# eth-cscs/COSTA

Measured on AMD Instinct MI355X. Metric: GB/s device-resident tile pack+transpose+unpack (fp64), % HBM peak, higher is better.
Workload: dtype f64; 1 GPU; pxtran fp64 16384x16384, 256x256 blocks, op T, alpha=1 beta=0, 1x1 grid (BASELINE configs[1]); op=T, parallelism=1 rank(s), one per GPU, RCCL send/recv exchange, m=16384, n=16384, block=256, grid=1x1

## Files before the change

### costa_amd/__init__.py

```python
from __future__ import annotations

import ctypes as C
import os
import struct
from dataclasses import dataclass
from typing import Iterable, Sequence

import numpy as np

__all__ = [
    "CostaError", "lib", "FLOAT", "DOUBLE", "CFLOAT", "CDOUBLE", "INT32", "dtype_code",
    "np_dtype", "Layout", "block_cyclic_layout", "custom_layout", "Comm", "transform",
    "transform_batch", "transform_async", "transform_batch_async", "synchronize", "transformer", "copy_and_transform", "execute_tiles", "execute_tiles_mixed",
    "convert_subtile", "TileOp",
    "plan_export", "set_profiling", "get_stats", "release_caches", "TILE_OP_DTYPE",
]

FLOAT, DOUBLE, CFLOAT, CDOUBLE, INT32 = 0, 1, 2, 3, 4
_NP = {FLOAT: np.float32, DOUBLE: np.float64, CFLOAT: np.complex64,
       CDOUBLE: np.complex128, INT32: np.int32}

TILE_TRANSPOSE, TILE_CONJ, TILE_VEC_SRC, TILE_VEC_DST = 0x1, 0x2, 0x4, 0x8
SCALE_BITCOPY, SCALE_ZERO, SCALE_ALPHA, SCALE_AXPBY = 0, 1, 2, 3

# ... 99 lines not shown
        "costa_hip_layout_num_blocks": (i, [vp]),
        "costa_hip_layout_block": (i, [vp, i, C.POINTER(i), C.POINTER(i), C.POINTER(i),
                                       C.POINTER(i), C.POINTER(vp), C.POINTER(i)]),
        "costa_hip_comm_self": (i, [i, C.POINTER(vp)]),
        "costa_hip_comm_unique_id": (i, [C.c_char_p]),
        "costa_hip_comm_create": (i, [C.c_char_p, i, i, i, C.POINTER(vp)]),
        "costa_hip_comm_rank": (i, [vp]),
        "costa_hip_comm_size": (i, [vp]),
        "costa_hip_comm_destroy": (None, [vp]),
        "costa_hip_transform": (i, [vp, vp, c, vp, vp, vp]),
        "costa_hip_transform_batch": (i, [i, C.POINTER(vp), C.POINTER(vp), C.c_char_p, vp, vp,
                                          vp]),
        "costa_hip_transform_async": (i, [vp, vp, c, vp, vp, vp, vp]),
        "costa_hip_transform_batch_async": (i, [i, C.POINTER(vp), C.POINTER(vp), C.c_char_p, vp,
                                                vp, vp, vp]),
        "costa_hip_synchronize": (i, [vp]),
        "costa_hip_device_count": (i, [C.POINTER(i)]),
        "costa_hip_rccl_version": (i, [C.POINTER(i)]),
        "costa_hip_copy_and_transform": (i, [i, i, i, vp, i, i, vp, i, i, i, i, vp, vp]),
        "costa_hip_execute_tiles": (i, [i, C.POINTER(TileOp), i64, vp, vp, vp, i, i]),
        "costa_hip_execute_tiles_mixed": (i, [i, i, C.POINTER(TileOp), i64, vp, vp, vp, i, i]),
        "costa_hip_convert_subtile": (i, [i, i, C.POINTER(i), C.POINTER(i)]),
        "costa_hip_plan_export": (i, [i, C.POINTER(vp), C.POINTER(vp), C.c_char_p, vp, vp, i, i,
                                      C.POINTER(PlanInfo), vp, vp, vp, vp, vp, vp, vp, vp]),
        "costa_hip_set_profiling": (i, [i]),
        "costa_hip_get_stats": (i, [C.POINTER(FullStats), i]),
        "costa_hip_release_caches": (i, []),
        "costa_hip_set_host_staging": (i, [i]),
        "costa_hip_set_planner": (i, [i]),
        "costa_hip_plan_export_device": (i, [i, i, C.POINTER(vp), C.POINTER(vp), C.c_char_p, vp, vp,
                                             i, i, C.POINTER(PlanInfo), vp, vp, vp, vp, vp, vp, vp,
                                             vp]),
        "costa_hip_set_list_builder": (i, [i]),
        "costa_hip_work_export": (i, [i, vp, i64, i, i, vp, i64, vp, i64, C.POINTER(i64)]),
    }
    for name, (res, args) in sig.items():
        f = getattr(L, name)
        f.restype = res
        f.argtypes = args
    _lib = L
    return L


def _check(rc: int):
    if rc != 0:
        raise CostaError(rc, lib().costa_hip_last_error().decode(errors="replace"))


def _ptr(p) -> int:
    if p is None:
        return 0
    if isinstance(p, int):
        return p
    if isinstance(p, np.ndarray):
        return p.ctypes.data
    if hasattr(p, "data_ptr"):
        return p.data_ptr()
    raise TypeError(f"cannot take the address of {type(p)}")


def _scalar_bytes(code: int, x) -> bytes:
    if code == DOUBLE:
        return struct.pack("<d", float(x))
    if code == CDOUBLE:
        z = complex(x)
        return struct.pack("<dd", z.real, z.imag)
# ... 4 lines not shown
    return C.c_char(x.encode()[:1])


@dataclass
class BlockInfo:
    row_start: int
    row_end: int
    col_start: int
    col_end: int
    data: int
    ld: int


class Layout:

    def __init__(self, handle: int, dtype: int, keep: Iterable = ()):
        self._h = C.c_void_p(handle)
        self.dtype = dtype
        self._keep = list(keep)

    @property
    def handle(self) -> C.c_void_p:
        return self._h

    def num_blocks(self) -> int:
        return lib().costa_hip_layout_num_blocks(self._h)

    def block(self, i: int) -> BlockInfo:
        v = [C.c_int() for _ in range(4)]
        d, ld = C.c_void_p(), C.c_int()
        _check(lib().costa_hip_layout_block(self._h, i, *[C.byref(x) for x in v], C.byref(d),
                                            C.byref(ld)))
        return BlockInfo(v[0].value, v[1].value, v[2].value, v[3].value, d.value or 0, ld.value)

    def reorder_ranks(self, reordering: Sequence[int]):
        p = np.ascontiguousarray(reordering, dtype=np.int32)
        _check(lib().costa_hip_layout_reorder_ranks(self._h, p.ctypes.data_as(C.POINTER(C.c_int)),
                                                    int(p.size)))

    def close(self):
        if self._h and self._h.value:
            lib().costa_hip_layout_destroy(self._h)
            self._h = C.c_void_p(0)

    def __del__(self):
        try:
            self.close()
        except Exception:
            pass


def block_cyclic_layout(m, n, block_m, block_n, i, j, sub_m, sub_n, p_m, p_n, order, rsrc, csrc,
                        ptr, lld, ordering, rank, dtype=DOUBLE) -> Layout:
    code = dtype_code(dtype)
    h = C.c_void_p()
    _check(lib().costa_hip_block_cyclic_layout(code, m, n, block_m, block_n, i, j, sub_m, sub_n,
                                               p_m, p_n, _chr(order), rsrc, csrc,
                                               C.c_void_p(_ptr(ptr)), lld, _chr(ordering), rank,
                                               C.byref(h)))
    return Layout(h.value, code, [ptr])


def custom_layout(rowblocks, colblocks, rowsplit, colsplit, owners, localblocks, ordering,
                  dtype=DOUBLE) -> Layout:
    code = dtype_code(dtype)
    rs = np.ascontiguousarray(rowsplit, dtype=np.int32)
# ... 208 lines not shown
        def export(*args):
            return L.costa_hip_plan_export_device(int(device), *args)
    _check(export(n, a, c, tb, ab, bb, rank, nranks, C.byref(info), None, None,
                  None, None, None, None, None, None))
    lo = np.zeros(info.n_local, TILE_OP_DTYPE)
    po = np.zeros(info.n_pack, TILE_OP_DTYPE)
    uo = np.zeros(info.n_unpack, TILE_OP_DTYPE)
    cnt = [np.zeros(nranks, np.int64) for _ in range(4)]
    sc = np.zeros(2 * info.n_slots, _NP[code])
    _check(export(n, a, c, tb, ab, bb, rank, nranks, C.byref(info),
                  lo.ctypes.data, po.ctypes.data, uo.ctypes.data,
                  *[x.ctypes.data for x in cnt], sc.ctypes.data))
    return Plan(lo, po, uo, *cnt, sc, info.send_elems, info.recv_elems, info.local_elems)


def set_profiling(on: bool = True):
    _check(lib().costa_hip_set_profiling(int(on)))


def get_stats(reset: bool = False) -> dict:
    s = FullStats()
    _check(lib().costa_hip_get_stats(C.byref(s), int(reset)))
    return s.as_dict()


def release_caches():
    _check(lib().costa_hip_release_caches())


def set_planner(mode: int):
    _check(lib().costa_hip_set_planner(int(mode)))


def set_list_builder(mode: int):
    _check(lib().costa_hip_set_list_builder(int(mode)))


@dataclass
class WorkLists:
    ordered: np.ndarray
    work: np.ndarray
    meta: dict
    on_gpu: bool


_WORK_META = ("n_large", "n_medium", "n_skew", "n_cblock", "cblock_lds", "cb_map", "tiny_first",
              "n_tiny", "n_ordered", "n_work", "on_gpu", "flags")


def work_export(dtype, ops: np.ndarray, kind: str = "local", device=None) -> WorkLists:
    code = dtype_code(dtype)
    ops = np.ascontiguousarray(ops, dtype=TILE_OP_DTYPE)
    k = {"local": 0, "pack": 1, "unpack": 2}[kind]
    dev = -1 if device is None else int(device)
    meta = (C.c_int64 * 12)()
    L = lib()
    _check(L.costa_hip_work_export(code, ops.ctypes.data, ops.size, k, dev, None, 0, None, 0, meta))
    o = np.zeros(meta[8], TILE_OP_DTYPE)
    w = np.zeros(meta[9], np.uint64)
    _check(L.costa_hip_work_export(code, ops.ctypes.data, ops.size, k, dev, o.ctypes.data, o.size,
                                   w.ctypes.data, w.size, meta))
    m = dict(zip(_WORK_META, list(meta)))
    return WorkLists(o, w, m, bool(m["on_gpu"]))


def set_host_staging(mode: int):
# ... 8 lines not shown
```

### costa_amd/csrc/capi.cpp

```cpp
#include "engine.hpp"

#include <hip/hip_runtime.h>

#include <costa/transform.hpp>

#include <algorithm>
#include <cctype>
#include <complex>
#include <cstring>
#include <new>

struct costa_layout_s {
    costa::engine::elayout e;
    std::vector<int> base_owners;
};
struct costa_comm_s {
    costa::engine::comm* c = nullptr;
};

namespace {
thread_local std::string g_last_error;

template <typename F>
int guarded(F&& f) {
// ... 346 lines not shown
        [&](const std::vector<job>& jobs) { return costa::engine::make_plan(jobs, rank, nranks); },
        n, A, C, trans, alpha, beta, rank, nranks, info, local_ops, pack_ops, unpack_ops,
        send_counts, send_displs, recv_counts, recv_displs, scalars);
}

int costa_hip_plan_export_device(int device, int n, const costa_layout_t* A, const costa_layout_t* C,
                                 const char* trans, const void* alpha, const void* beta, int rank,
                                 int nranks, costa_plan_info_t* info, costa_tile_op_t* local_ops,
                                 costa_tile_op_t* pack_ops, costa_tile_op_t* unpack_ops,
                                 int64_t* send_counts, int64_t* send_displs, int64_t* recv_counts,
                                 int64_t* recv_displs, void* scalars) {
    device_restore keep;
    return export_plan(
        [&](const std::vector<job>& jobs) {
            auto p = costa::engine::make_plan_device(jobs, rank, nranks, 0, device, nullptr);
            if (!p)
                throw costa::engine::error(COSTA_ERR_ARG,
                                           "costa: the device planner does not apply to these "
                                           "layouts (local blocks are not exactly the rank's grid "
                                           "cells)");
            return p;
        },
        n, A, C, trans, alpha, beta, rank, nranks, info, local_ops, pack_ops, unpack_ops,
        send_counts, send_displs, recv_counts, recv_displs, scalars);
}

int costa_hip_set_planner(int mode) {
    return guarded([&] {
        if (mode < 0 || mode > 2) throw costa::engine::error(COSTA_ERR_ARG, "mode must be 0, 1 or 2");
        costa::engine::set_planner_mode(mode);
    });
}

int costa_hip_set_list_builder(int mode) {
    return guarded([&] {
        if (mode < 0 || mode > 2) throw costa::engine::error(COSTA_ERR_ARG, "mode must be 0, 1 or 2");
        costa::engine::set_list_builder_mode(mode);
    });
}

int costa_hip_work_export(int dtype, const costa_tile_op_t* ops, int64_t n_ops, int kind, int device,
                          costa_tile_op_t* ordered, int64_t cap_ordered, uint64_t* work,
                          int64_t cap_work, int64_t* meta) {
    auto body = [&] {
        if (!meta || (n_ops > 0 && !ops) || n_ops < 0) throw costa::engine::error(COSTA_ERR_ARG, "null argument");
        if (dtype < COSTA_FLOAT || dtype > COSTA_INT32) throw costa::engine::error(COSTA_ERR_ARG, "bad dtype");
        if (kind < 0 || kind > 2) throw costa::engine::error(COSTA_ERR_ARG, "kind must be 0, 1 or 2");
        std::vector<costa_tile_op_t> in(ops, ops + n_ops), o;
        std::vector<uint64_t> w;
        costa::engine::work_split ws;
        const bool on_gpu = costa::engine::work_export(
            costa_dtype_t(dtype), in, costa::engine::list_kind(kind), device, o, w, ws);
        const int64_t m[12] = {ws.n_large, ws.n_medium, ws.n_skew, ws.n_cblock, ws.cblock_lds, ws.cb_map,
                               ws.tiny_first, ws.n_tiny, int64_t(o.size()), int64_t(w.size()), on_gpu,
                               int64_t(ws.tr_shape) | int64_t(ws.sq) << 1 | int64_t(ws.full) << 2 |
                                   int64_t(ws.med_full) << 3 | int64_t(ws.med_sq) << 4 |
                                   int64_t(ws.skew_wide) << 5};
        std::memcpy(meta, m, sizeof(m));
        if (ordered && cap_ordered >= int64_t(o.size()) && !o.empty())
            std::memcpy(ordered, o.data(), o.size() * sizeof(o[0]));
        if (work && cap_work >= int64_t(w.size()) && !w.empty()) std::memcpy(work, w.data(), w.size() * sizeof(w[0]));
    };
    return device >= 0 ? gpu_guarded(body) : guarded(body);
}

int costa_hip_set_profiling(int on) {
// ... 138 lines not shown
```

### costa_amd/csrc/engine.cpp

```cpp
#include <exception>
#include <thread>
#include "engine.hpp"

#include <hip/hip_runtime.h>
#include <rccl/rccl.h>

#include <algorithm>
#include <numeric>
#include <chrono>
#include <cmath>
#include <cstdio>
#include <cstdlib>
#include <cstring>
#include <deque>
#include <list>
#include <map>
#include <mutex>
#include <unordered_map>

namespace costa {
namespace engine {

#define HIP_CHECK(x)                                                                   \
    do {                                                                               \
// ... 1347 lines not shown
        if (d) {
            hipDeviceptr_t base = nullptr;
            size_t sz = 0;
            if (hipMemGetAddressRange(&base, &sz, const_cast<char*>(b.data)) == hipSuccess) {
                lo = reinterpret_cast<uintptr_t>(base);
                hi = lo + sz;
            } else {
                (void)hipGetLastError();
            }
        }
    }
    return first;
}

}

namespace {
int g_host_mode = -1;
}
int host_staging_mode() {
    if (g_host_mode < 0) {
        const char* s = std::getenv("COSTA_HOST_STAGING");
        g_host_mode = s ? (std::atoi(s) != 0) : 1;
    }
    return g_host_mode;
}
void set_host_staging_mode(int mode) {
    std::lock_guard<std::recursive_mutex> lk(g_mutex);
    g_host_mode = mode != 0;
}

namespace {

struct hasher {
    uint64_t h = 0x9E3779B97F4A7C15ull;
    uint64_t h2 = 0x2545F4914F6CDD1Dull;
    void mix(uint64_t v) {
        v ^= v >> 33;
        v *= 0xff51afd7ed558ccdull;
        v ^= v >> 33;
        h = (h ^ v) * 0xc4ceb9fe1a85ec53ull + 0x165667b19e3779f9ull;
        h ^= h >> 29;
        h2 = (h2 + v) * 0x9fb21c651e98df25ull;
        h2 ^= h2 >> 31;
    }
    void mix_vec(const std::vector<int>& v) {
        mix(v.size());
        for (int x : v) mix(uint64_t(uint32_t(x)));
    }
    void mix_layout(const elayout& L) {
        mix(uint64_t(L.dtype));
        mix(uint64_t(uint8_t(L.ordering)));
        mix(uint64_t(L.n_ranks));
        mix_vec(L.rows_split);
        mix_vec(L.cols_split);
        mix_vec(L.owners);
        mix(L.blocks.size());
        for (const auto& b : L.blocks) {
            mix(uint64_t(uint32_t(b.rows.start)) | (uint64_t(uint32_t(b.rows.end)) << 32));
            mix(uint64_t(uint32_t(b.cols.start)) | (uint64_t(uint32_t(b.cols.end)) << 32));
            mix(reinterpret_cast<uintptr_t>(b.data));
            mix(uint64_t(uint32_t(b.ld)));
        }
    }
};

}

uint64_t layout_hash(const elayout& L) {
    hasher h;
    h.mix_layout(L);
    return h.h | 1;
}

void layout_hashes(const elayout& L, uint64_t& h1, uint64_t& h2) {
    hasher h;
    h.mix_layout(L);
    h1 = h.h | 1;
    h2 = h.h2;
}

void set_layout_hash(elayout& L) { layout_hashes(L, L.hash, L.hash2); }

namespace {

struct cached_plan {
    std::unique_ptr<plan> p;
    int device = 0;
    bool staged = false;
    std::vector<hrange> h2d_ranges, d2h_ranges;
    dbuf stage;
    dbuf d_local, w_local, d_scal;
    work_split l_local;
    bool tr_local = true, ax_local = true;
    convert_list c_local;
    struct xround {
        dbuf d_pack, w_pack, d_unpack, w_unpack;
        work_split l_pack, l_unpack;
        convert_list c_pack, c_unpack;
        bool tr_unpack = false, ax_unpack = false;
    };
    std::vector<std::unique_ptr<xround>> rounds;
    std::vector<unsigned char> scal_host;
    std::shared_ptr<host_pipeline> pipe;
};

constexpr size_t kMaxPlans = 16;
struct keyed_plan {
    uint64_t h = 0;
    std::vector<uint64_t> key;
    std::unique_ptr<cached_plan> plan;
};
std::list<keyed_plan> g_plans;

void key_layout(std::vector<uint64_t>& k, const elayout& L) {
    uint64_t h1 = L.hash, h2 = L.hash2;
    if (!h1) layout_hashes(L, h1, h2);
    k.push_back(h1);
    k.push_back(h2);
    k.push_back(uint64_t(L.dtype) | uint64_t(uint8_t(L.ordering)) << 8 |
                uint64_t(uint32_t(L.n_ranks)) << 32);
    k.push_back(uint64_t(uint32_t(L.nbr())) | uint64_t(uint32_t(L.nbc())) << 32);
    k.push_back(L.blocks.size());
    if (!L.blocks.empty())
        for (const eblock* b : {&L.blocks.front(), &L.blocks.back()}) {
            k.push_back(reinterpret_cast<uintptr_t>(b->data));
            k.push_back(uint64_t(uint32_t(b->ld)) | uint64_t(uint32_t(b->rows.start)) << 32);
        }
}

elayout remap(const elayout& L, const std::vector<hrange>& ranges, char* dev) {
    elayout out = L;
    for (auto& b : out.blocks) {
        uintptr_t p = reinterpret_cast<uintptr_t>(b.data);
        auto it = std::upper_bound(ranges.begin(), ranges.end(), p,
                                   [](uintptr_t v, const hrange& r) { return v < r.lo; });
        if (it == ranges.begin()) throw error(COSTA_ERR_INTERNAL, "costa: staging map miss");
        --it;
        b.data = dev + it->dev_off + (p - it->lo);
    }
    return out;
}

std::vector<hrange> collect_ranges(const std::vector<const elayout*>& Ls) {
    std::vector<hrange> r;
    for (const elayout* L : Ls) {
        const size_t E = dtype_size(L->dtype);
        for (const auto& b : L->blocks) {
            size_t ext = block_extent_bytes(b, L->ordering, E);
            if (!ext) continue;
            uintptr_t lo = reinterpret_cast<uintptr_t>(b.data);
            r.push_back({lo, lo + ext, 0});
        }
    }
    std::sort(r.begin(), r.end(), [](const hrange& x, const hrange& y) { return x.lo < y.lo; });
    std::vector<hrange> m;
    for (const auto& x : r) {
        if (!m.empty() && x.lo <= m.back().hi)
            m.back().hi = std::max(m.back().hi, x.hi);
        else
            m.push_back(x);
    }
    return m;
}

}

namespace {
int g_planner = -1;
constexpr size_t kDevicePlanBlocks = 4096;
constexpr size_t kColdDevicePlanBlocks = 100000;
bool g_device_planner_warm = false;
}

int planner_mode() {
    if (g_planner < 0) {
        const char* s = std::getenv("COSTA_PLANNER");
        g_planner = s ? std::max(0, std::min(2, std::atoi(s))) : 1;
    }
    return g_planner;
}

void set_planner_mode(int mode) {
    std::lock_guard<std::recursive_mutex> lk(g_mutex);
    g_planner = mode;
}

namespace {
int g_list_builder = -1;
}

int list_builder_mode() {
    if (g_list_builder < 0) {
        const char* s = std::getenv("COSTA_LIST_BUILDER");
        g_list_builder = s ? std::max(0, std::min(2, std::atoi(s))) : 1;
    }
    return g_list_builder;
}

void set_list_builder_mode(int mode) {
    std::lock_guard<std::recursive_mutex> lk(g_mutex);
    g_list_builder = mode;
}

namespace {
template <typename X>
void upload_list(dbuf& d, const std::vector<X>& h, const X* sec, size_t at, size_t n, hipStream_t s) {
    if (!sec || n == 0) return d.upload(h, s);
    const size_t total = h.size() + n;
    d.reserve(total * sizeof(X));
    X* p = static_cast<X*>(d.p);
    if (at) HIP_CHECK(hipMemcpyAsync(p, h.data(), at * sizeof(X), hipMemcpyHostToDevice, s));
    HIP_CHECK(hipMemcpyAsync(p + at, sec, n * sizeof(X), hipMemcpyDeviceToDevice, s));
    if (h.size() > at)
        HIP_CHECK(hipMemcpyAsync(p + at + n, h.data() + at, (h.size() - at) * sizeof(X), hipMemcpyHostToDevice, s));
}
}

// ... 8 lines not shown
    device_section sec;
    sec.device = device;
    sec.stream = dc.main;
    sec.force = true;
    w = build_work(dtype, ops, ordered, work, kind, &sec);
    if (!sec.n_ordered) return false;
    std::vector<costa_tile_op_t> o(sec.n_ordered);
    std::vector<uint64_t> k(sec.n_work);
    HIP_CHECK(hipMemcpyAsync(o.data(), sec.d_ordered, o.size() * sizeof(o[0]), hipMemcpyDeviceToHost, dc.main));
    HIP_CHECK(hipMemcpyAsync(k.data(), sec.d_work, k.size() * sizeof(k[0]), hipMemcpyDeviceToHost, dc.main));
    HIP_CHECK(hipStreamSynchronize(dc.main));
    ordered.insert(ordered.begin() + std::ptrdiff_t(sec.at_ordered), o.begin(), o.end());
    work.insert(work.begin() + std::ptrdiff_t(sec.at_work), k.begin(), k.end());
    return true;
}

namespace {
std::unique_ptr<plan> plan_jobs(const std::vector<job>& jobs, comm* c, hipStream_t s) {
    const int lb = c->size == 1 && c->nccl ? loopback_exchange() : 0;
    const int mode = planner_mode();
    size_t blocks = 0;
    for (const job& j : jobs) blocks += j.A->blocks.size() + j.C->blocks.size();
    const size_t need = g_device_planner_warm ? kDevicePlanBlocks : kColdDevicePlanBlocks;
    if (mode == 2 || (mode == 1 && blocks >= need)) {
        if (auto p = make_plan_device(jobs, c->rank, c->size, lb, c->device, s)) {
            g_stats.device_plans++;
            g_device_planner_warm = true;
            return p;
        }
    }
    return make_plan(jobs, c->rank, c->size, lb);
}

cached_plan* get_plan(const std::vector<job>& jobs, comm* c, device_ctx& dc) {
    std::vector<uint64_t> key;
    key.reserve(4 + jobs.size() * 30);
    key.push_back(uint64_t(uint32_t(c->rank)) | uint64_t(uint32_t(c->size)) << 32);
    key.push_back(uint64_t(uint32_t(c->device)) | uint64_t(uint32_t(host_staging_mode())) << 32);
    key.push_back(jobs.size());
    for (const auto& j : jobs) {
        key_layout(key, *j.A);
        key_layout(key, *j.C);
        uint64_t w = uint64_t(uint8_t(std::toupper(static_cast<unsigned char>(j.trans))));
        for (bool cm : {true, false})
            w = w << 8 | scale_kind(j.C->dtype, j.s, cm, std::toupper(j.trans) == 'C');
        key.push_back(w);
    }
    hasher h;
    for (uint64_t w : key) h.mix(w);
    for (auto it = g_plans.begin(); it != g_plans.end(); ++it) {
        if (it->h == h.h && it->key == key) {
            g_plans.splice(g_plans.begin(), g_plans, it);
            g_stats.plan_hits++;
            return g_plans.front().plan.get();
        }
    }
    g_stats.plan_misses++;
    static const bool trace = std::getenv("COSTA_PLAN_TRACE") != nullptr;
    auto now = [] {
        return std::chrono::duration<double, std::milli>(
                   std::chrono::steady_clock::now().time_since_epoch()).count();
    };
    const double t0 = now();
    double t_resid = 0, t_plan = 0, t_work = 0;

    const bool mixed = any_mixed(jobs);
    if (mixed) {
        costa_dtype_t a, b;
        check_jobs(jobs, c->size, a, b);
    }
    auto cp = std::make_unique<cached_plan>();
    cp->device = c->device;
    bool all_dev = true;
    std::vector<const elayout*> host_layouts;
    std::vector<bool> on_dev;
    for (const auto& j : jobs)
        for (const elayout* L : {j.A, j.C}) {
            bool d = layout_on_device(*L);
            on_dev.push_back(d);
            all_dev = all_dev && d;
        }
    std::vector<elayout> remapped;
    std::vector<job> pj = jobs;
    std::vector<hrange> staged_ranges;
    std::vector<uint8_t> range_flags;
    if (!all_dev && mixed)
        throw error(COSTA_ERR_ARG,
                    "costa: mixed-precision transforms (A and C of different element types) need "
// ... 27 lines not shown
            for (int side = 0; side < 2; ++side) {
                if (!(side == 0 ? a_host : c_host)) continue;
                const elayout* L = side == 0 ? jobs[t].A : jobs[t].C;
                const size_t E = dtype_size(L->dtype);
                for (const auto& b : L->blocks) {
                    if (!block_extent_bytes(b, L->ordering, E)) continue;
                    const size_t i = range_of(reinterpret_cast<uintptr_t>(b.data));
                    if (side == 0) {
                        range_flags[i] |= 1;
                    } else {
                        range_flags[i] |= 2;
                        if (c_job[i] >= 0 && c_job[i] != int(t)) range_flags[i] |= 4;
                        c_job[i] = int(t);
                    }
                }
            }
        }
        bool pipe_ok = host_staging_mode() == 1 &&
                       std::none_of(on_dev.begin(), on_dev.end(), [](bool d) { return d; });
        for (uint8_t f : range_flags)
            if ((f & 3) == 3 || (f & 4)) pipe_ok = false;
        if (pipe_ok) {
            const double tp = now();
            auto hplan = plan_jobs(jobs, c, dc.main);
            g_stats.plan_ms += now() - tp;
            if (host_pipeline_accepts(hplan->dtype, hplan->pack_ops)) {
                cp->staged = false;
                cp->p = std::move(hplan);
                const int R = c->nccl ? exchange_rounds() : 1;
                std::vector<int> pr, ur;
                exchange_round_of_ops(*cp->p, R, pr, ur);
                cp->pipe = make_host_pipeline(cp->p->dtype, cp->p->pack_ops, cp->p->local_ops,
                                              cp->p->unpack_ops, pr, ur, R);
                g_plans.push_front({h.h, std::move(key), std::move(cp)});
                while (g_plans.size() > kMaxPlans) g_plans.pop_back();
                return g_plans.front().plan.get();
            }
        }
        cp->stage.reserve(std::max<size_t>(off, 256));
        staged_ranges = ranges;
        remapped.reserve(jobs.size() * 2);
        k = 0;
        for (auto& j : pj) {
            if (!on_dev[k++]) {
                remapped.push_back(remap(*j.A, ranges, static_cast<char*>(cp->stage.p)));
                j.A = &remapped.back();
            }
            if (!on_dev[k++]) {
                remapped.push_back(remap(*j.C, ranges, static_cast<char*>(cp->stage.p)));
                j.C = &remapped.back();
            }
        }
    }
    t_resid = now() - t0;
    cp->p = plan_jobs(pj, c, dc.main);
    const plan& p = *cp->p;
    t_plan = now() - t0 - t_resid;
    g_stats.plan_ms += t_plan;
    if (cp->staged) {
        const size_t E = dtype_size(p.dtype);
        const uintptr_t base = reinterpret_cast<uintptr_t>(cp->stage.p);
        std::vector<size_t> written(staged_ranges.size(), 0);
        std::vector<bool> reads_c(staged_ranges.size(), false);
        auto account = [&](const std::vector<costa_tile_op_t>& ops) {
            for (const auto& op : ops) {
                if (op.dst < base) continue;
                const size_t off = size_t(op.dst - base);
// ... 52 lines not shown
        x->ax_unpack = any_axpby(up[size_t(r)]);
        if (cv_pack)
            x->c_pack = build_convert_work(p.src_dtype, p.pkg_dtype, pk[size_t(r)], 0, 0, ord_p[size_t(r)],
                                           w_p[size_t(r)]);
        else
            x->l_pack = build_work(p.pkg_dtype, pk[size_t(r)], ord_p[size_t(r)], w_p[size_t(r)], list_pack);
        if (cv_unpack)
            x->c_unpack = build_convert_work(p.pkg_dtype, p.dtype, up[size_t(r)], 0, 0, ord_u[size_t(r)],
                                             w_u[size_t(r)]);
        else
            x->l_unpack = build_work(p.dtype, up[size_t(r)], ord_u[size_t(r)], w_u[size_t(r)], list_unpack,
                                     &sec_u[size_t(r)]);
        cp->rounds.push_back(std::move(x));
    }
    t_work = now() - t0 - t_resid - t_plan;
    upload_list(cp->d_local, ord_l, sec_l.d_ordered, sec_l.at_ordered, sec_l.n_ordered, dc.main);
    upload_list(cp->w_local, w_l, sec_l.d_work, sec_l.at_work, sec_l.n_work, dc.main);
    for (int r = 0; r < R; ++r) {
        auto& x = *cp->rounds[size_t(r)];
        const device_section& su = sec_u[size_t(r)];
        x.d_pack.upload(ord_p[size_t(r)], dc.main);
        x.w_pack.upload(w_p[size_t(r)], dc.main);
        upload_list(x.d_unpack, ord_u[size_t(r)], su.d_ordered, su.at_ordered, su.n_ordered, dc.main);
        upload_list(x.w_unpack, w_u[size_t(r)], su.d_work, su.at_work, su.n_work, dc.main);
    }
    HIP_CHECK(hipStreamSynchronize(dc.main));
    if (trace)
        std::fprintf(stderr,
                     "[costa plan] %zu local / %zu pack / %zu unpack ops: residency %.2f ms, "
                     "planning %.2f, work lists %.2f, upload %.2f, total %.2f\n",
                     p.local_ops.size(), p.pack_ops.size(), p.unpack_ops.size(), t_resid, t_plan,
                     t_work, now() - t0 - t_resid - t_plan - t_work, now() - t0);

    g_plans.push_front({h.h, std::move(key), std::move(cp)});
    while (g_plans.size() > kMaxPlans) g_plans.pop_back();
    return g_plans.front().plan.get();
}

void upload_scalars(cached_plan& cp, const std::vector<job>& jobs, hipStream_t s) {
    const size_t E = dtype_size(cp.p->dtype);
    std::vector<unsigned char> host(jobs.size() * 2 * E);
    for (size_t t = 0; t < jobs.size(); ++t) {
        std::memcpy(&host[(2 * t) * E], jobs[t].s.alpha.data(), E);
        std::memcpy(&host[(2 * t + 1) * E], jobs[t].s.beta.data(), E);
    }
    if (host != cp.scal_host || !cp.d_scal.p) {
        cp.d_scal.reserve(host.size());
        cp.scal_host = host;
        HIP_CHECK(hipMemcpyAsync(cp.d_scal.p, cp.scal_host.data(), host.size(),
                                 hipMemcpyHostToDevice, s));
    }
}

}

void release_caches() {
    std::lock_guard<std::recursive_mutex> lk(g_mutex);
    g_plans.clear();
    release_host_rings();
    ctx_map().clear();
}

namespace {
enum phase { PH_LOCAL, PH_PACK, PH_EXCHANGE, PH_UNPACK, PH_H2D, PH_D2H };

struct phase_timer {
    device_ctx& dc;
// ... 62 lines not shown
    device_ctx& dc = ctx(c->device);
    HIP_CHECK(hipStreamSynchronize(dc.main));
    HIP_CHECK(hipStreamSynchronize(dc.aux));
    HIP_CHECK(hipStreamSynchronize(dc.xch));
    dc.resolve();
}

namespace {
void issue_exchange(comm* c, const plan& p, char* sb, char* rb, hipStream_t s, int round = 0,
                    int rounds = 1) {
    const size_t E = dtype_size(p.pkg_dtype);
    const size_t piece = max_message_bytes();
    NCCL_CHECK(ncclGroupStart());
    for (int q = 0; q < c->size; ++q) {
        int64_t slo, shi, rlo, rhi;
        round_range(p.send_counts[size_t(q)], E, rounds, round, slo, shi);
        round_range(p.recv_counts[size_t(q)], E, rounds, round, rlo, rhi);
        const size_t sbytes = size_t(shi - slo) * E, rbytes = size_t(rhi - rlo) * E;
        char* sp = sb + size_t(p.send_displs[size_t(q)] + slo) * E;
        char* rp = rb + size_t(p.recv_displs[size_t(q)] + rlo) * E;
        for (size_t o = 0; o < sbytes; o += piece)
            NCCL_CHECK(ncclSend(sp + o, std::min(piece, sbytes - o), ncclUint8, q, c->nccl, s));
        for (size_t o = 0; o < rbytes; o += piece)
            NCCL_CHECK(ncclRecv(rp + o, std::min(piece, rbytes - o), ncclUint8, q, c->nccl, s));
    }
    NCCL_CHECK(ncclGroupEnd());
}
}

void transform(const std::vector<job>& jobs, comm* c, void* user_stream, bool async) {
    std::lock_guard<std::recursive_mutex> lk(g_mutex);
    if (!c) throw error(COSTA_ERR_ARG, "costa: null communicator");
    device_ctx& dc = ctx(c->device);
    cached_plan& cp = *get_plan(jobs, c, dc);
    const plan& p = *cp.p;
    const size_t E = dtype_size(p.pkg_dtype);
    if (async && (cp.staged || cp.pipe))
        throw error(COSTA_ERR_ARG,
                    "costa: asynchronous transforms need device-resident layouts (host data is "
                    "staged synchronously)");
    hipStream_t user = static_cast<hipStream_t>(user_stream);
    if (user) {
        HIP_CHECK(hipEventRecord(dc.ev_user, user));
        HIP_CHECK(hipStreamWaitEvent(dc.main, dc.ev_user, 0));
    }
    upload_scalars(cp, jobs, dc.main);
    if (cp.pipe) {
        const bool xchg = c->nccl != nullptr && (p.send_elems > 0 || p.recv_elems > 0);
        char *sb = nullptr, *rb = nullptr;
        std::function<void(void*, int)> fn;
        if (xchg) {
            dc.send.reserve(size_t(p.send_elems) * E + 256);
            dc.recv.reserve(size_t(p.recv_elems) * E + 256);
            sb = static_cast<char*>(dc.send.p);
            rb = static_cast<char*>(dc.recv.p);
            const int R = exchange_rounds();
            fn = [&, R](void* s, int r) {
                issue_exchange(c, p, sb, rb, static_cast<hipStream_t>(s), r, R);
            };
        }
        HIP_CHECK(hipEventRecord(dc.ev_ready, dc.main));
        HIP_CHECK(hipStreamWaitEvent(dc.aux, dc.ev_ready, 0));
        run_host_pipeline(*cp.pipe, c->device, dc.aux, dc.main, sb, rb, fn, cp.d_scal.p);
        g_stats.transforms++;
        return;
    }
    phase_timer tm(dc, g_profiling);

    if (cp.staged) {
        tm.start(PH_H2D, dc.main);
        for (const auto& r : cp.h2d_ranges)
            HIP_CHECK(hipMemcpyAsync(static_cast<char*>(cp.stage.p) + r.dev_off,
                                     reinterpret_cast<void*>(r.lo), r.hi - r.lo,
                                     hipMemcpyHostToDevice, dc.main));
        tm.stop();
    }

    const bool exchange = c->nccl != nullptr && (p.send_elems > 0 || p.recv_elems > 0);
    hipStream_t ls = exchange ? dc.aux : dc.main;
    if (exchange) {
        HIP_CHECK(hipEventRecord(dc.ev_ready, dc.main));
        HIP_CHECK(hipStreamWaitEvent(dc.aux, dc.ev_ready, 0));
    }
    if (cp.c_local.n_items) {
        tm.start(PH_LOCAL, ls);
        launch_convert(p.src_dtype, p.dtype, static_cast<const costa_tile_op_t*>(cp.d_local.p),
                       static_cast<const uint64_t*>(cp.w_local.p), cp.c_local, nullptr, nullptr,
                       cp.d_scal.p, ls);
        tm.stop();
    }
    if (cp.l_local.n_items()) {
        tm.start(PH_LOCAL, ls);
        launch_tiles(p.dtype,
                     make_launch(cp.l_local, cp.d_local.p, cp.w_local.p, nullptr, nullptr,
                                 cp.d_scal.p, cp.tr_local, cp.ax_local),
                     ls);
        tm.stop();
    }

    if (exchange) {
        dc.send.reserve(size_t(p.send_elems) * E + 256);
        dc.recv.reserve(size_t(p.recv_elems) * E + 256);
        char* sb = static_cast<char*>(dc.send.p);
        char* rb = static_cast<char*>(dc.recv.p);
        const int R = int(cp.rounds.size());
        dc.round_events(size_t(R));
        for (int r = 0; r < R; ++r) {
            const auto& x = *cp.rounds[size_t(r)];
            if (x.c_pack.n_items) {
                tm.start(PH_PACK, dc.main);
                launch_convert(p.src_dtype, p.pkg_dtype, static_cast<const costa_tile_op_t*>(x.d_pack.p),
                               static_cast<const uint64_t*>(x.w_pack.p), x.c_pack, nullptr, sb,
                               cp.d_scal.p, dc.main);
                tm.stop();
            }
            if (x.l_pack.n_items()) {
                tm.start(PH_PACK, dc.main);
                launch_tiles(p.pkg_dtype,
                             make_launch(x.l_pack, x.d_pack.p, x.w_pack.p, nullptr, sb, cp.d_scal.p,
                                         false, false),
                             dc.main);
                tm.stop();
            }
            HIP_CHECK(hipEventRecord(dc.ev_packed[size_t(r)], dc.main));
            HIP_CHECK(hipStreamWaitEvent(dc.xch, dc.ev_packed[size_t(r)], 0));
            tm.start(PH_EXCHANGE, dc.xch);
            issue_exchange(c, p, sb, rb, dc.xch, r, R);
            tm.stop();
            HIP_CHECK(hipEventRecord(dc.ev_moved[size_t(r)], dc.xch));
        }
        for (int r = 0; r < R; ++r) {
            const auto& x = *cp.rounds[size_t(r)];
            if (x.c_unpack.n_items) {
                HIP_CHECK(hipStreamWaitEvent(dc.aux, dc.ev_moved[size_t(r)], 0));
                tm.start(PH_UNPACK, dc.aux);
                launch_convert(p.pkg_dtype, p.dtype, static_cast<const costa_tile_op_t*>(x.d_unpack.p),
                               static_cast<const uint64_t*>(x.w_unpack.p), x.c_unpack, rb, nullptr,
                               cp.d_scal.p, dc.aux);
                tm.stop();
            }
            if (!x.l_unpack.n_items()) continue;
            HIP_CHECK(hipStreamWaitEvent(dc.aux, dc.ev_moved[size_t(r)], 0));
            tm.start(PH_UNPACK, dc.aux);
            launch_tiles(p.dtype,
                         make_launch(x.l_unpack, x.d_unpack.p, x.w_unpack.p, rb, nullptr,
                                     cp.d_scal.p, x.tr_unpack, x.ax_unpack),
                         dc.aux);
            tm.stop();
        }
        HIP_CHECK(hipEventRecord(dc.ev_local, dc.aux));
        HIP_CHECK(hipStreamWaitEvent(dc.main, dc.ev_local, 0));
        HIP_CHECK(hipStreamWaitEvent(dc.main, dc.ev_moved[size_t(R - 1)], 0));
    }

    if (cp.staged) {
        tm.start(PH_D2H, dc.main);
        for (const auto& r : cp.d2h_ranges)
            HIP_CHECK(hipMemcpyAsync(reinterpret_cast<void*>(r.lo),
                                     static_cast<char*>(cp.stage.p) + r.dev_off, r.hi - r.lo,
                                     hipMemcpyDeviceToHost, dc.main));
        tm.stop();
    }

    g_stats.transforms++;
    auto count_items = [&](const work_split& w) {
        g_stats.tile_items += w.n_large + w.n_medium;
        g_stats.skew_items += w.n_skew;
        g_stats.cblock_items += w.n_cblock;
        g_stats.tiny_items += w.n_tiny;
        if (!dtype_is_complex(p.dtype) && pieces_in_group_launch(w.n_cblock, w.n_tiny))
            g_stats.fused_pieces += w.n_tiny;
    };
    if (cp.l_local.n_items() || cp.c_local.n_items) {
        g_stats.local_launches++;
        g_stats.local_bytes += p.local_bytes;
        count_items(cp.l_local);
        g_stats.convert_items += cp.c_local.n_items;
    }
// ... 108 lines not shown
```

### costa_amd/csrc/engine.hpp

```cpp
#pragma once

#include <costa/layout.hpp>
#include <costa_hip.h>

#include <array>
#include <cstdint>
#include <functional>
#include <memory>
#include <string>
#include <vector>

namespace costa {
namespace engine {

size_t dtype_size(costa_dtype_t t);
bool dtype_is_complex(costa_dtype_t t);

struct eblock {
    interval rows, cols;
    char* data = nullptr;
    int ld = 0;
};

struct elayout {
    costa_dtype_t dtype = COSTA_DOUBLE;
    std::vector<int> rows_split, cols_split;
    std::vector<int> owners;
    int n_ranks = 1;
    char ordering = 'C';
    std::vector<eblock> blocks;
    uint64_t hash = 0;
    uint64_t hash2 = 0;

    int nbr() const { return int(rows_split.size()) - 1; }
    int nbc() const { return int(cols_split.size()) - 1; }
};

template <typename T>
costa_dtype_t dtype_of();

template <typename T>
elayout erase(const grid_layout<T>& L);

uint64_t layout_hash(const elayout& L);
void layout_hashes(const elayout& L, uint64_t& h1, uint64_t& h2);
void set_layout_hash(elayout& L);

struct scal {
    std::array<unsigned char, 16> alpha{};
    std::array<unsigned char, 16> beta{};
};

struct job {
    const elayout* A = nullptr;
    const elayout* C = nullptr;
    char trans = 'N';
    scal s;
};

struct plan {
    costa_dtype_t dtype = COSTA_DOUBLE;
    costa_dtype_t src_dtype = COSTA_DOUBLE;
    costa_dtype_t pkg_dtype = COSTA_DOUBLE;
    bool mixed() const { return src_dtype != dtype; }
    int rank = 0, n_ranks = 1;
    std::vector<costa_tile_op_t> local_ops, pack_ops, unpack_ops;
    std::vector<int64_t> send_counts, send_displs, recv_counts, recv_displs;
    int64_t send_elems = 0, recv_elems = 0, local_elems = 0;
    std::vector<scal> slots;
    int64_t local_bytes = 0, pack_bytes = 0, unpack_bytes = 0;
};

struct job_params {
    bool transpose, conj, a_cm, c_cm;
    uint32_t kind_copy, kind_tr;
};
std::vector<job_params> check_jobs(const std::vector<job>& jobs, int n_ranks, costa_dtype_t& dtype);
std::vector<job_params> check_jobs(const std::vector<job>& jobs, int n_ranks,
                                   costa_dtype_t& src_dtype, costa_dtype_t& dst_dtype);
const char* dtype_name(costa_dtype_t t);
bool any_mixed(const std::vector<job>& jobs);

std::unique_ptr<plan> make_plan(const std::vector<job>& jobs, int rank, int n_ranks,
                                int loopback = 0);

std::unique_ptr<plan> make_plan_device(const std::vector<job>& jobs, int rank, int n_ranks,
                                       int loopback, int device, void* stream);
int planner_mode();
void set_planner_mode(int mode);

int loopback_exchange();

const char* tuning_env(const char* name);

size_t max_message_bytes();

int exchange_rounds();

costa_tile_op_t make_tile_op(int n_rows, int n_cols, uint64_t src, int src_stride, bool src_cm,
                             uint64_t dst, int dst_stride, bool dst_cm, bool transpose, bool conj,
                             uint32_t scale_kind, uint32_t slot, size_t elem);
costa_tile_op_t make_tile_op(int n_rows, int n_cols, uint64_t src, int src_stride, bool src_cm,
                             uint64_t dst, int dst_stride, bool dst_cm, bool transpose, bool conj,
                             uint32_t scale_kind, uint32_t slot, size_t src_elem, size_t dst_elem);

uint32_t scale_kind(costa_dtype_t dtype, const scal& s, bool copy_mode, bool conj);

int device_count();
int rccl_version();
struct comm;
struct comm* comm_self(int device);
struct comm* comm_create(const unsigned char* id, int nranks, int rank, int device);
void comm_unique_id(unsigned char* out);
int comm_rank(const struct comm* c);
int comm_size(const struct comm* c);
void comm_destroy(struct comm* c);

void transform(const std::vector<job>& jobs, struct comm* c, void* user_stream = nullptr,
               bool async = false);
void synchronize(struct comm* c);
void resolve_pending();

// ... 153 lines not shown
```

### include/costa_hip.h

```cpp
#ifndef COSTA_HIP_H
#define COSTA_HIP_H

#include <stddef.h>
#include <stdint.h>

#ifdef __cplusplus
extern "C" {
#endif

#define COSTA_OK 0
#define COSTA_ERR_ARG 1
#define COSTA_ERR_HIP 2
#define COSTA_ERR_NCCL 3
#define COSTA_ERR_INTERNAL 4

typedef enum {
    COSTA_FLOAT = 0,
    COSTA_DOUBLE = 1,
    COSTA_CFLOAT = 2,
    COSTA_CDOUBLE = 3,
    COSTA_INT32 = 4
} costa_dtype_t;

typedef struct costa_layout_s* costa_layout_t;
// ... 98 lines not shown
                          int64_t* send_counts, int64_t* send_displs, int64_t* recv_counts,
                          int64_t* recv_displs, void* scalars);

typedef struct {
    double pack_ms, local_ms, unpack_ms, exchange_ms, h2d_ms, d2h_ms;
    int64_t pack_launches, local_launches, unpack_launches;
    int64_t pack_bytes, local_bytes, unpack_bytes;
    int64_t transforms;
    int64_t plan_hits, plan_misses;
    int64_t host_groups;
    int64_t device_plans;
    double plan_ms;
    int64_t host_direct;
    int64_t host_direct_groups;
    int64_t tile_items, skew_items, cblock_items, tiny_items;
    int64_t device_lists;
    int64_t fused_pieces;
    int64_t convert_items;
} costa_stats_t;
int costa_hip_set_profiling(int on);
int costa_hip_get_stats(costa_stats_t* out, int reset);
int costa_hip_release_caches(void);

int costa_hip_set_host_staging(int mode);

int costa_hip_set_planner(int mode);
int costa_hip_plan_export_device(int device, int n, const costa_layout_t* A, const costa_layout_t* C,
                                 const char* trans, const void* alpha, const void* beta, int rank,
                                 int nranks, costa_plan_info_t* info, costa_tile_op_t* local_ops,
                                 costa_tile_op_t* pack_ops, costa_tile_op_t* unpack_ops,
                                 int64_t* send_counts, int64_t* send_displs, int64_t* recv_counts,
                                 int64_t* recv_displs, void* scalars);

int costa_hip_set_list_builder(int mode);
int costa_hip_work_export(int dtype, const costa_tile_op_t* ops, int64_t n_ops, int kind, int device,
                          costa_tile_op_t* ordered, int64_t cap_ordered, uint64_t* work,
                          int64_t cap_work, int64_t* meta);

#ifdef __cplusplus
}
#endif
#endif
```

Baseline: 6220 GB/s.

## Cache transform plans by base-relative layout and rebase pointers at launch

Layout hashes and plan keys now use block offsets relative to the first block instead of absolute pointers. When a layout with the same shape is resident on the device at a different address, the cached plan is reused and the kernels receive source and destination base offsets. This avoids rebuilding plans when buffers are reallocated between calls. The cost is extra key computation, a small memo of verified base pairs, and an overlap check between source and destination spans. It is enabled by default through an environment toggle.

```diff
diff --git a/costa_amd/__init__.py b/costa_amd/__init__.py
--- a/costa_amd/__init__.py
+++ b/costa_amd/__init__.py
@@ -155,6 +155,8 @@
                                              i, i, C.POINTER(PlanInfo), vp, vp, vp, vp, vp, vp, vp,
                                              vp]),
         "costa_hip_set_list_builder": (i, [i]),
+        "costa_hip_set_plan_rebase": (i, [i]),
+        "costa_hip_layout_hash": (i, [vp, C.POINTER(C.c_uint64), C.POINTER(C.c_uint64)]),
         "costa_hip_work_export": (i, [i, vp, i64, i, i, vp, i64, vp, i64, C.POINTER(i64)]),
     }
     for name, (res, args) in sig.items():
@@ -225,6 +227,11 @@
         _check(lib().costa_hip_layout_block(self._h, i, *[C.byref(x) for x in v], C.byref(d),
                                             C.byref(ld)))
         return BlockInfo(v[0].value, v[1].value, v[2].value, v[3].value, d.value or 0, ld.value)
+
+    def content_hash(self):
+        h1, h2 = C.c_uint64(), C.c_uint64()
+        _check(lib().costa_hip_layout_hash(self._h, C.byref(h1), C.byref(h2)))
+        return h1.value, h2.value
 
     def reorder_ranks(self, reordering: Sequence[int]):
         p = np.ascontiguousarray(reordering, dtype=np.int32)
@@ -499,6 +506,10 @@
     _check(lib().costa_hip_set_planner(int(mode)))
 
 
+def set_plan_rebase(on: bool):
+    _check(lib().costa_hip_set_plan_rebase(1 if on else 0))
+
+
 def set_list_builder(mode: int):
     _check(lib().costa_hip_set_list_builder(int(mode)))
 
diff --git a/costa_amd/csrc/capi.cpp b/costa_amd/csrc/capi.cpp
--- a/costa_amd/csrc/capi.cpp
+++ b/costa_amd/csrc/capi.cpp
@@ -402,6 +402,21 @@
     });
 }
 
+int costa_hip_set_plan_rebase(int on) {
+    return guarded([&] {
+        if (on != 0 && on != 1) throw costa::engine::error(COSTA_ERR_ARG, "on must be 0 or 1");
+        costa::engine::set_plan_rebase_mode(on);
+    });
+}
+
+int costa_hip_layout_hash(costa_layout_t layout, uint64_t* h1, uint64_t* h2) {
+    return guarded([&] {
+        if (!layout || !h1 || !h2) throw costa::engine::error(COSTA_ERR_ARG, "null argument");
+        *h1 = layout->e.hash;
+        *h2 = layout->e.hash2;
+    });
+}
+
 int costa_hip_set_list_builder(int mode) {
     return guarded([&] {
         if (mode < 0 || mode > 2) throw costa::engine::error(COSTA_ERR_ARG, "mode must be 0, 1 or 2");
diff --git a/costa_amd/csrc/engine.cpp b/costa_amd/csrc/engine.cpp
--- a/costa_amd/csrc/engine.cpp
+++ b/costa_amd/csrc/engine.cpp
@@ -1403,6 +1403,10 @@
 
 namespace {
 
+uintptr_t layout_base(const elayout& L) {
+    return L.blocks.empty() ? 0 : reinterpret_cast<uintptr_t>(L.blocks.front().data);
+}
+
 struct hasher {
     uint64_t h = 0x9E3779B97F4A7C15ull;
     uint64_t h2 = 0x2545F4914F6CDD1Dull;
@@ -1427,10 +1431,11 @@
         mix_vec(L.cols_split);
         mix_vec(L.owners);
         mix(L.blocks.size());
+        const uintptr_t base = layout_base(L);
         for (const auto& b : L.blocks) {
             mix(uint64_t(uint32_t(b.rows.start)) | (uint64_t(uint32_t(b.rows.end)) << 32));
             mix(uint64_t(uint32_t(b.cols.start)) | (uint64_t(uint32_t(b.cols.end)) << 32));
-            mix(reinterpret_cast<uintptr_t>(b.data));
+            mix(reinterpret_cast<uintptr_t>(b.data) - base);
             mix(uint64_t(uint32_t(b.ld)));
         }
     }
@@ -1451,7 +1456,21 @@
     h2 = h.h2;
 }
 
-void set_layout_hash(elayout& L) { layout_hashes(L, L.hash, L.hash2); }
+void layout_span(const elayout& L, int64_t& lo, int64_t& hi) {
+    lo = hi = 0;
+    const size_t E = dtype_size(L.dtype);
+    const uintptr_t base = layout_base(L);
+    for (const auto& b : L.blocks) {
+        const int64_t o = int64_t(reinterpret_cast<uintptr_t>(b.data) - base);
+        lo = std::min(lo, o);
+        hi = std::max(hi, o + int64_t(block_extent_bytes(b, L.ordering, E)));
+    }
+}
+
+void set_layout_hash(elayout& L) {
+    layout_hashes(L, L.hash, L.hash2);
+    layout_span(L, L.span_lo, L.span_hi);
+}
 
 namespace {
 
@@ -1474,6 +1493,20 @@
     std::vector<std::unique_ptr<xround>> rounds;
     std::vector<unsigned char> scal_host;
     std::shared_ptr<host_pipeline> pipe;
+    uintptr_t a_base = 0, c_base = 0;
+    static constexpr size_t kMemo = 64;
+    std::array<std::pair<uintptr_t, uintptr_t>, kMemo> memo{};
+    size_t n_memo = 0, memo_next = 0;
+    bool memo_has(uintptr_t a, uintptr_t c) const {
+        for (size_t i = 0; i < n_memo; ++i)
+            if (memo[i].first == a && memo[i].second == c) return true;
+        return false;
+    }
+    void memo_add(uintptr_t a, uintptr_t c) {
+        memo[memo_next] = {a, c};
+        memo_next = (memo_next + 1) % kMemo;
+        n_memo = std::min(n_memo + 1, kMemo);
+    }
 };
 
 constexpr size_t kMaxPlans = 16;
@@ -1484,9 +1517,17 @@
 };
 std::list<keyed_plan> g_plans;
 
-void key_layout(std::vector<uint64_t>& k, const elayout& L) {
+struct layout_at {
+    uintptr_t base, lo, hi;
+};
+layout_at key_layout(std::vector<uint64_t>& k, const elayout& L) {
     uint64_t h1 = L.hash, h2 = L.hash2;
-    if (!h1) layout_hashes(L, h1, h2);
+    int64_t s_lo = L.span_lo, s_hi = L.span_hi;
+    if (!h1) {
+        layout_hashes(L, h1, h2);
+        layout_span(L, s_lo, s_hi);
+    }
+    const uintptr_t base = layout_base(L);
     k.push_back(h1);
     k.push_back(h2);
     k.push_back(uint64_t(L.dtype) | uint64_t(uint8_t(L.ordering)) << 8 |
@@ -1495,9 +1536,10 @@
     k.push_back(L.blocks.size());
     if (!L.blocks.empty())
         for (const eblock* b : {&L.blocks.front(), &L.blocks.back()}) {
-            k.push_back(reinterpret_cast<uintptr_t>(b->data));
+            k.push_back(reinterpret_cast<uintptr_t>(b->data) - base);
             k.push_back(uint64_t(uint32_t(b->ld)) | uint64_t(uint32_t(b->rows.start)) << 32);
         }
+    return {base, base + uintptr_t(s_lo), base + uintptr_t(s_hi)};
 }
 
 elayout remap(const elayout& L, const std::vector<hrange>& ranges, char* dev) {
@@ -1555,6 +1597,23 @@
 void set_planner_mode(int mode) {
     std::lock_guard<std::recursive_mutex> lk(g_mutex);
     g_planner = mode;
+}
+
+namespace {
+int g_plan_rebase = -1;
+}
+
+int plan_rebase_mode() {
+    if (g_plan_rebase < 0) {
+        const char* s = std::getenv("COSTA_PLAN_REBASE");
+        g_plan_rebase = s ? (std::atoi(s) != 0) : 1;
+    }
+    return g_plan_rebase;
+}
+
+void set_plan_rebase_mode(int mode) {
+    std::lock_guard<std::recursive_mutex> lk(g_mutex);
+    g_plan_rebase = mode != 0;
 }
 
 namespace {
@@ -1629,28 +1688,81 @@
     return make_plan(jobs, c->rank, c->size, lb);
 }
 
-cached_plan* get_plan(const std::vector<job>& jobs, comm* c, device_ctx& dc) {
-    std::vector<uint64_t> key;
-    key.reserve(4 + jobs.size() * 30);
+cached_plan* get_plan(const std::vector<job>& jobs, comm* c, device_ctx& dc, const char*& d_src,
+                      char*& d_dst) {
+    d_src = nullptr;
+    d_dst = nullptr;
+    const bool rebase = plan_rebase_mode() != 0;
+    std::vector<uint64_t> key, abs_tail, reb_tail;
+    key.reserve(8 + jobs.size() * 36);
     key.push_back(uint64_t(uint32_t(c->rank)) | uint64_t(uint32_t(c->size)) << 32);
     key.push_back(uint64_t(uint32_t(c->device)) | uint64_t(uint32_t(host_staging_mode())) << 32);
     key.push_back(jobs.size());
-    for (const auto& j : jobs) {
-        key_layout(key, *j.A);
-        key_layout(key, *j.C);
+    uintptr_t a0 = 0, c0 = 0;
+    uintptr_t a_lo = ~uintptr_t(0), a_hi = 0, c_lo = ~uintptr_t(0), c_hi = 0;
+    for (size_t t = 0; t < jobs.size(); ++t) {
+        const job& j = jobs[t];
+        const layout_at la = key_layout(key, *j.A);
+        const layout_at lc = key_layout(key, *j.C);
         uint64_t w = uint64_t(uint8_t(std::toupper(static_cast<unsigned char>(j.trans))));
         for (bool cm : {true, false})
             w = w << 8 | scale_kind(j.C->dtype, j.s, cm, std::toupper(j.trans) == 'C');
         key.push_back(w);
-    }
-    hasher h;
-    for (uint64_t w : key) h.mix(w);
-    for (auto it = g_plans.begin(); it != g_plans.end(); ++it) {
-        if (it->h == h.h && it->key == key) {
-            g_plans.splice(g_plans.begin(), g_plans, it);
-            g_stats.plan_hits++;
-            return g_plans.front().plan.get();
-        }
+        abs_tail.push_back(la.base);
+        abs_tail.push_back(lc.base);
+        if (!rebase) continue;
+        if (t == 0) a0 = la.base, c0 = lc.base;
+        reb_tail.push_back(la.base % kRebaseAlign | (lc.base % kRebaseAlign) << 32);
+        if (t > 0) {
+            reb_tail.push_back(la.base - a0);
+            reb_tail.push_back(lc.base - c0);
+        }
+        if (la.hi > la.lo) a_lo = std::min(a_lo, la.lo), a_hi = std::max(a_hi, la.hi);
+        if (lc.hi > lc.lo) c_lo = std::min(c_lo, lc.lo), c_hi = std::max(c_hi, lc.hi);
+    }
+    const bool overlap = rebase && a_lo < c_hi && c_lo < a_hi;
+    if (overlap) reb_tail.push_back(c0 - a0);
+    auto find = [&](const std::vector<uint64_t>& k, uint64_t h) -> cached_plan* {
+        for (auto it = g_plans.begin(); it != g_plans.end(); ++it)
+            if (it->h == h && it->key == k) {
+                g_plans.splice(g_plans.begin(), g_plans, it);
+                return g_plans.front().plan.get();
+            }
+        return nullptr;
+    };
+    auto finish = [](std::vector<uint64_t> k, uint64_t tag, const std::vector<uint64_t>& tail, uint64_t& h) {
+        k.push_back(tag);
+        k.insert(k.end(), tail.begin(), tail.end());
+        hasher hs;
+        for (uint64_t w : k) hs.mix(w);
+        h = hs.h;
+        return k;
+    };
+    uint64_t h_reb = 0, h_abs = 0;
+    std::vector<uint64_t> key_reb;
+    bool resident = false;
+    if (rebase) {
+        key_reb = finish(key, overlap ? 2 : 1, reb_tail, h_reb);
+        if (cached_plan* cp = find(key_reb, h_reb)) {
+            resident = cp->memo_has(a0, c0);
+            if (!resident) {
+                resident = true;
+                for (const auto& j : jobs)
+                    resident = resident && layout_on_device(*j.A) && layout_on_device(*j.C);
+                if (resident) cp->memo_add(a0, c0);
+            }
+            if (resident) {
+                g_stats.plan_hits++;
+                d_src = reinterpret_cast<const char*>(a0 - cp->a_base);
+                d_dst = reinterpret_cast<char*>(c0 - cp->c_base);
+                return cp;
+            }
+        }
+    }
+    key = finish(std::move(key), 0, abs_tail, h_abs);
+    if (cached_plan* cp = find(key, h_abs)) {
+        g_stats.plan_hits++;
+        return cp;
     }
     g_stats.plan_misses++;
     static const bool trace = std::getenv("COSTA_PLAN_TRACE") != nullptr;
@@ -1744,7 +1856,7 @@
                 exchange_round_of_ops(*cp->p, R, pr, ur);
                 cp->pipe = make_host_pipeline(cp->p->dtype, cp->p->pack_ops, cp->p->local_ops,
                                               cp->p->unpack_ops, pr, ur, R);
-                g_plans.push_front({h.h, std::move(key), std::move(cp)});
+                g_plans.push_front({h_abs, std::move(key), std::move(cp)});
                 while (g_plans.size() > kMaxPlans) g_plans.pop_back();
                 return g_plans.front().plan.get();
             }
@@ -1863,7 +1975,14 @@
                      p.local_ops.size(), p.pack_ops.size(), p.unpack_ops.size(), t_resid, t_plan,
                      t_work, now() - t0 - t_resid - t_plan - t_work, now() - t0);
 
-    g_plans.push_front({h.h, std::move(key), std::move(cp)});
+    if (rebase && all_dev) {
+        cp->a_base = a0;
+        cp->c_base = c0;
+        cp->memo_add(a0, c0);
+        g_plans.push_front({h_reb, std::move(key_reb), std::move(cp)});
+    } else {
+        g_plans.push_front({h_abs, std::move(key), std::move(cp)});
+    }
     while (g_plans.size() > kMaxPlans) g_plans.pop_back();
     return g_plans.front().plan.get();
 }
@@ -1992,7 +2111,9 @@
     std::lock_guard<std::recursive_mutex> lk(g_mutex);
     if (!c) throw error(COSTA_ERR_ARG, "costa: null communicator");
     device_ctx& dc = ctx(c->device);
-    cached_plan& cp = *get_plan(jobs, c, dc);
+    const char* d_src = nullptr;
+    char* d_dst = nullptr;
+    cached_plan& cp = *get_plan(jobs, c, dc, d_src, d_dst);
     const plan& p = *cp.p;
     const size_t E = dtype_size(p.pkg_dtype);
     if (async && (cp.staged || cp.pipe))
@@ -2045,14 +2166,14 @@
     if (cp.c_local.n_items) {
         tm.start(PH_LOCAL, ls);
         launch_convert(p.src_dtype, p.dtype, static_cast<const costa_tile_op_t*>(cp.d_local.p),
-                       static_cast<const uint64_t*>(cp.w_local.p), cp.c_local, nullptr, nullptr,
+                       static_cast<const uint64_t*>(cp.w_local.p), cp.c_local, d_src, d_dst,
                        cp.d_scal.p, ls);
         tm.stop();
     }
     if (cp.l_local.n_items()) {
         tm.start(PH_LOCAL, ls);
         launch_tiles(p.dtype,
-                     make_launch(cp.l_local, cp.d_local.p, cp.w_local.p, nullptr, nullptr,
+                     make_launch(cp.l_local, cp.d_local.p, cp.w_local.p, d_src, d_dst,
                                  cp.d_scal.p, cp.tr_local, cp.ax_local),
                      ls);
         tm.stop();
@@ -2070,14 +2191,14 @@
             if (x.c_pack.n_items) {
                 tm.start(PH_PACK, dc.main);
                 launch_convert(p.src_dtype, p.pkg_dtype, static_cast<const costa_tile_op_t*>(x.d_pack.p),
-                               static_cast<const uint64_t*>(x.w_pack.p), x.c_pack, nullptr, sb,
+                               static_cast<const uint64_t*>(x.w_pack.p), x.c_pack, d_src, sb,
                                cp.d_scal.p, dc.main);
                 tm.stop();
             }
             if (x.l_pack.n_items()) {
                 tm.start(PH_PACK, dc.main);
                 launch_tiles(p.pkg_dtype,
-                             make_launch(x.l_pack, x.d_pack.p, x.w_pack.p, nullptr, sb, cp.d_scal.p,
+                             make_launch(x.l_pack, x.d_pack.p, x.w_pack.p, d_src, sb, cp.d_scal.p,
                                          false, false),
                              dc.main);
                 tm.stop();
@@ -2095,7 +2216,7 @@
                 HIP_CHECK(hipStreamWaitEvent(dc.aux, dc.ev_moved[size_t(r)], 0));
                 tm.start(PH_UNPACK, dc.aux);
                 launch_convert(p.pkg_dtype, p.dtype, static_cast<const costa_tile_op_t*>(x.d_unpack.p),
-                               static_cast<const uint64_t*>(x.w_unpack.p), x.c_unpack, rb, nullptr,
+                               static_cast<const uint64_t*>(x.w_unpack.p), x.c_unpack, rb, d_dst,
                                cp.d_scal.p, dc.aux);
                 tm.stop();
             }
@@ -2103,7 +2224,7 @@
             HIP_CHECK(hipStreamWaitEvent(dc.aux, dc.ev_moved[size_t(r)], 0));
             tm.start(PH_UNPACK, dc.aux);
             launch_tiles(p.dtype,
-                         make_launch(x.l_unpack, x.d_unpack.p, x.w_unpack.p, rb, nullptr,
+                         make_launch(x.l_unpack, x.d_unpack.p, x.w_unpack.p, rb, d_dst,
                                      cp.d_scal.p, x.tr_unpack, x.ax_unpack),
                          dc.aux);
             tm.stop();
diff --git a/costa_amd/csrc/engine.hpp b/costa_amd/csrc/engine.hpp
--- a/costa_amd/csrc/engine.hpp
+++ b/costa_amd/csrc/engine.hpp
@@ -31,6 +31,7 @@
     std::vector<eblock> blocks;
     uint64_t hash = 0;
     uint64_t hash2 = 0;
+    int64_t span_lo = 0, span_hi = 0;
 
     int nbr() const { return int(rows_split.size()) - 1; }
     int nbc() const { return int(cols_split.size()) - 1; }
@@ -44,6 +45,7 @@
 
 uint64_t layout_hash(const elayout& L);
 void layout_hashes(const elayout& L, uint64_t& h1, uint64_t& h2);
+void layout_span(const elayout& L, int64_t& lo, int64_t& hi);
 void set_layout_hash(elayout& L);
 
 struct scal {
@@ -88,6 +90,10 @@
                                        int loopback, int device, void* stream);
 int planner_mode();
 void set_planner_mode(int mode);
+
+constexpr uint64_t kRebaseAlign = 256;
+int plan_rebase_mode();
+void set_plan_rebase_mode(int mode);
 
 int loopback_exchange();
 
diff --git a/include/costa_hip.h b/include/costa_hip.h
--- a/include/costa_hip.h
+++ b/include/costa_hip.h
@@ -154,6 +154,9 @@
                                  int64_t* send_counts, int64_t* send_displs, int64_t* recv_counts,
                                  int64_t* recv_displs, void* scalars);
 
+int costa_hip_set_plan_rebase(int on);
+int costa_hip_layout_hash(costa_layout_t layout, uint64_t* h1, uint64_t* h2);
+
 int costa_hip_set_list_builder(int mode);
 int costa_hip_work_export(int dtype, const costa_tile_op_t* ops, int64_t n_ops, int kind, int device,
                           costa_tile_op_t* ordered, int64_t cap_ordered, uint64_t* work,
```

Result: no change. 6222 GB/s, median of 3 (+0.0%).
